# fudan-zvg/S-NeRF

Measured on AMD Instinct MI355X. Metric: rays/sec (train step), higher is better.
Workload: dtype bf16; 1 GPU; S-NeRF path A (MipNerfModel) train step, nuScenes-like 1600x900 rays, 64 proposal + 128 fine evals/ray (192 spp), hidden 1024, rgb_layer 3, cone + contraction + IPE-96

## Files before the change

include/snerf_hip.h:

```cpp
#ifndef SNERF_HIP_H
#define SNERF_HIP_H
#ifdef __cplusplus
extern "C" {
#endif

#define SNERF_DT_F32 0
#define SNERF_DT_BF16 1
#define SNERF_DT_F16 2
#define SNERF_DT_F64 3
#define SNERF_DT_BF16X3 4
#define SNERF_ACT_NONE 0
#define SNERF_ACT_RELU 1
#define SNERF_ACT_MASK 2
#define SNERF_ACT_RELU_BITS 3
#define SNERF_ACT_MASK_BITS 4

int snerf_version(void);
int snerf_last_hip_error(void);
int snerf_debug_lds_scribble(int seed, void* stream);

int snerf_linear_fwd(const void* A, long lda, const void* W, long ldw, const float* bias, void* Y, long ldy,
                     const void* aux, long ldaux, float* colsum, float* colsum_ws, int M, int N, int K, int n_store,
                     int act, int dtype, int out_f32, int variant, void* stream);

// ... 94 lines not shown
                            const float* dirs, long R, int S, int opaque, float bg, float rgb_padding, float density_bias,
                            float* rgb, float* depth, float* acc, float* weights, void* stream);
int snerf_zip_composite_bwd(const float* raw_rgb, long ld_rgb, const float* raw_density, long ld_den, const float* tdist,
                            const float* dirs, long R, int S, int opaque, float bg, float rgb_padding, float density_bias,
                            const float* weights, const float* acc, const float* depth, const float* g_rgb, const float* g_depth,
                            const float* g_acc, const float* g_w, float* d_raw_rgb, long ld_drgb, float* d_raw_density,
                            long ld_dden, float* g_dirs, void* stream);

int snerf_adam_step(float* p, float* g, float* m, float* v, long n, float lr, float b1, float b2, float eps, int step,
                    float grad_scale, int zero_grad, void* stream);
int snerf_app_embed(const float* emb, const float* app, int n_vocab, long n_rays, int S, int dim, void* dst, long ld, int dtype,
                    const int* sample_id, long rows, void* stream);
int snerf_app_embed_bwd(const float* dV, long ld, const float* app, int n_vocab, long n_rays, int S, int dim, float* g_emb, void* stream);
int snerf_app_embed_bwd_det(const float* dV, long ld, const float* app, int n_vocab, long n_rays, int S, int dim, float* g_emb, void* stream);
int snerf_index_check(const float* idx, long n, int n_rows, int* bad, void* stream);

int snerf_split_cast(const float* src, long ld_src, long M, int C, int Cpad, void* dst, long ld_dst, void* stream);

#define SNERF_DT_F16F8 5
int snerf_split8_cast(const float* src, long ld_src, long M, int C, int Cpad, void* dst, long ld_dst, int weight, void* stream);

int snerf_colsum_f32(const float* x, long ld, long M, int C, float* out, void* stream);
int snerf_cast_pad(const float* src, long ld_src, long M, int C, int Cpad, void* dst, long ld_dst, int dtype, void* stream);
int snerf_classic_x_grad(const float* g0, long ld0, const float* g5, long ld5, const float* gv, long ldv, long M, int ic, int icv,
                         float* dx, long ld_dx, void* stream);
int snerf_gather_pack(const float* flat, const int* idx, long n, void* dst, int dtype, void* stream);
int snerf_gather_pack_tiles(const float* flat, const int* idx, long n, void* dst, int dtype, const int* tiles, int n_tiles, void* stream);
int snerf_gather_pack_pair(const float* flat, const int* idx, long n, void* dst, int dtype, const int* tiles, int n_tiles, const int* idx32,
                           long n32, float* dst32, void* stream);

int snerf_semantic_composite_fwd(const float* weights, const void* logits, long ld, int dtype, long R, int S, int C, int softmax,
                                 const int* row_index, float* sem, void* stream);
int snerf_semantic_composite_bwd(const float* weights, const void* logits, long ld, int dtype, const float* g_sem, long R, int S, int C,
                                 int softmax, float* d_logits, long ld_d, float* g_w_out, void* stream);

int snerf_ert_compact(const float* s0, const float* w0, const float* s1, long N, int S0, int S1, float eps_t, float eps_w,
                      void* masks, int* counts, int* row_index, int* sample_id, long* total, void* stream);
int snerf_ert_f2b_step(const float* prev_raw_d, long ld_den, long prev_base, const float* s1, const float* dirs, const float* near,
                       const float* far, long N, int S1, int g0, int G, int next_g0, int next_G, int transform_idx, float density_bias,
                       float eps_t, float* tau, int* flags, int* counts, int* row_index, int* sample_id, long row_base, long* total,
                       void* stream);
int snerf_classic_ert_step(const float* raw_g, int C, const int* alive, long n, const float* z_all, int S, const float* rays, long ld_rays,
                           int g0, int G, float eps_t, float* T, float* raw_full, int* keep, int* offs, int* alive_next, long* total,
                           void* stream);
int snerf_classic_ert_points(const float* rays, long ld_rays, const float* z_all, int S, const int* alive, long n, int g0, int G,
                             float* pts, float* viewdirs, int viewdir_col, void* stream);
// ... 243 lines not shown
```

snerf_amd/_lib.py:

```python
import ctypes
import os
import re

_HERE = os.path.dirname(os.path.abspath(__file__))
_REPO = os.path.dirname(_HERE)
LIB_PATH = os.environ.get("SNERF_HIP_LIB") or os.path.join(_HERE, "lib", "libsnerf_hip.so")
HEADER_PATH = os.path.join(_REPO, "include", "snerf_hip.h")
IO_LIB_PATH = os.path.join(_HERE, "lib", "libsnerf_io.so")
IO_HEADER_PATH = os.path.join(_REPO, "include", "snerf_io.h")

_CTYPE = {"int": ctypes.c_int, "long": ctypes.c_long, "float": ctypes.c_float, "double": ctypes.c_double}
RESTYPE = {}
_lib = None
_iolib = None


def parse_header(path: str = HEADER_PATH):
    src = open(path).read()
    src = re.sub(r"/\*.*?\*/", " ", src, flags=re.S)
    protos = {}
    for m in re.finditer(r"\b(int|long)\s+(snerf_\w+)\s*\(([^)]*)\)\s*;", src):
        name, args = m.group(2), m.group(3).strip()
        RESTYPE[name] = _CTYPE[m.group(1)]
        sig = []
        if args and args != "void":
            for a in args.split(","):
                a = " ".join(a.split())
                if "*" in a:
                    sig.append((ctypes.c_void_p, a.split("*")[-1].strip()))
                else:
                    ty, an = a.rsplit(" ", 1)
                    sig.append((_CTYPE[ty.replace("const ", "").strip()], an))
        protos[name] = sig
    return protos


def load():
    global _lib
    if _lib is not None:
        return _lib
    import torch
    if not os.path.exists(LIB_PATH):
        raise RuntimeError(
            f"libsnerf_hip.so not found at {LIB_PATH}: build it with `python -c 'import __graft_entry__ as g; g.build()'` "
            "(or `make -C snerf_amd/csrc`).  snerf_amd has no CPU/PyTorch fallback for its kernels.")
    lib = ctypes.CDLL(LIB_PATH)
    for name, sig in parse_header().items():
        fn = getattr(lib, name)
        fn.argtypes = [t for t, _ in sig]
        fn.restype = RESTYPE[name]
    _lib = lib
    return lib


def load_io():
    global _iolib
    if _iolib is not None:
        return _iolib
    if not os.path.exists(IO_LIB_PATH):
        raise RuntimeError(f"libsnerf_io.so not found at {IO_LIB_PATH}: build it with `make -C snerf_amd/csrc`")
    lib = ctypes.CDLL(IO_LIB_PATH)
    for name, sig in parse_header(IO_HEADER_PATH).items():
        fn = getattr(lib, name)
        fn.argtypes = [t for t, _ in sig]
        fn.restype = ctypes.c_long if name == "snerf_png_encode" else ctypes.c_int
    _iolib = lib
    return lib


class SnerfHipError(RuntimeError):
    pass


_STATUS = {1: "bad argument", 2: "kernel launch failure"}


def query(name: str, *args):
    return getattr(load(), name)(*args)


def call(name: str, *args):
    rc = getattr(load(), name)(*args)
    if rc != 0:
        extra = f", hipError_t {load().snerf_last_hip_error()}" if rc == 2 else ""
        raise SnerfHipError(f"{name} failed: status {rc} ({_STATUS.get(rc, 'unknown')}{extra})")
```

snerf_amd/csrc/common.h:

```cpp
#pragma once
#include <hip/hip_runtime.h>
#include <stdint.h>

#define SNERF_OK 0
#define SNERF_ERR_ARG 1
#define SNERF_ERR_LAUNCH 2

typedef __attribute__((ext_vector_type(8))) __bf16 bf16x8;
typedef __attribute__((ext_vector_type(4))) __bf16 bf16x4;
typedef __attribute__((ext_vector_type(8))) _Float16 h16x8;
typedef __attribute__((ext_vector_type(16))) float f32x16;
typedef __attribute__((ext_vector_type(4))) float f32x4;

#define SNERF_DT_F32 0
#define SNERF_DT_BF16 1
#define SNERF_DT_F16 2
#define SNERF_DT_F64 3
#define SNERF_DT_BF16X3 4
#define SNERF_DT_F16F8 5

extern int g_snerf_last_hip_error;
static inline int snerf_check_launch() {
  hipError_t e = hipGetLastError();
  if (e != hipSuccess) g_snerf_last_hip_error = (int)e;
  return e == hipSuccess ? SNERF_OK : SNERF_ERR_LAUNCH;
}

template <auto Kernel> static inline void snerf_raise_lds_limit(int limit) {
  static const hipError_t raised = hipFuncSetAttribute((const void*)Kernel, hipFuncAttributeMaxDynamicSharedMemorySize, limit);
  (void)raised;
}
template <auto Kernel, typename... Args>
static inline void snerf_launch(dim3 grid, dim3 block, size_t lds, int limit, hipStream_t stream, const Args&... args) {
  snerf_raise_lds_limit<Kernel>(limit);
  hipLaunchKernelGGL(Kernel, grid, block, lds, stream, args...);
}

static inline int snerf_cu_count() {
  static const int n_cu = [] {
    int dev = 0, n = 0;
    hipDeviceProp_t prop;
    if (hipGetDevice(&dev) == hipSuccess && hipGetDeviceProperties(&prop, dev) == hipSuccess) n = prop.multiProcessorCount;
    return n > 0 ? n : 256;
  }();
  return n_cu;
}

__device__ __forceinline__ int xcd_remap(int bid, int nblk) {
  const int q = nblk >> 3, r = nblk & 7;
  const int xcd = bid & 7, idx = bid >> 3;
  const int base = xcd < r ? xcd * (q + 1) : r * (q + 1) + (xcd - r) * q;
  return base + idx;
}

__device__ __forceinline__ float wave_sum(float v) {
#pragma unroll
  for (int o = 32; o > 0; o >>= 1) v += __shfl_xor(v, o, 64);
  return v;
}
// ... 46 lines not shown
```

snerf_amd/csrc/elementwise.hip:

```cpp
#include "common.h"

struct AdamArgs {
  float lr, b1, b2, eps, grad_scale, grad_max_val;
  int zero_grad, nonfinite;
  const int* step_dev;
  const float* lr_dev;
  const float* clip_coef;
  int step;
  unsigned long long* dropped;
};

__device__ __forceinline__ float adam_clean_grad(float g, const AdamArgs& a, float coef) {
  g *= a.grad_scale * coef;
  if (a.grad_max_val > 0.f && g == g) g = fminf(fmaxf(g, -a.grad_max_val), a.grad_max_val);
  if (a.nonfinite == 1) g = (fabsf(g) <= 3.402823466e+38f) ? g : 0.f;
  else if (a.nonfinite == 2) g = (g != g) ? 0.f : fminf(fmaxf(g, -3.402823466e+38f), 3.402823466e+38f);
  return g;
}

__device__ __forceinline__ void adam_update(float& p, float& m, float& v, float gk, float b1, float b2, float step_size, float bc2_sqrt, float eps) {
#pragma clang fp contract(off)
  m = b1 * m + (1.f - b1) * gk;
  v = b2 * v + ((1.f - b2) * gk) * gk;
  p = p - (step_size * m) / (sqrtf(v) / bc2_sqrt + eps);
// ... 509 lines not shown
      (n_tiles > 0 && (tiles == nullptr || (((uintptr_t)tiles) & 15)))) return SNERF_ERR_ARG;
  if (n_b < 0 || (n_b > 0 && (idx_b == nullptr || dst_b == nullptr || (((uintptr_t)idx_b) & 15)))) return SNERF_ERR_ARG;
  const long want = (n + 1023) / 1024, want_b = (n_b + 1023) / 1024;
  const int gblocks = (int)(want < 4096 ? want : 4096), tblocks = (n_tiles + 3) / 4, bblocks = (int)(want_b < 1024 ? want_b : 1024);
  const dim3 g((unsigned)(gblocks + tblocks + bblocks)), b(256);
  const PackTile* tl = (const PackTile*)tiles;
  hipStream_t s = (hipStream_t)stream;
  if (dtype == SNERF_DT_F32) hipLaunchKernelGGL(gather_pack_tiles_kernel<float>, g, b, 0, s, flat, idx, n, (float*)dst, tl, n_tiles, tblocks, gblocks, idx_b, n_b, dst_b);
  else if (dtype == SNERF_DT_BF16) hipLaunchKernelGGL(gather_pack_tiles_kernel<__bf16>, g, b, 0, s, flat, idx, n, (__bf16*)dst, tl, n_tiles, tblocks, gblocks, idx_b, n_b, dst_b);
  else if (dtype == SNERF_DT_F16) hipLaunchKernelGGL(gather_pack_tiles_kernel<_Float16>, g, b, 0, s, flat, idx, n, (_Float16*)dst, tl, n_tiles, tblocks, gblocks, idx_b, n_b, dst_b);
  else return SNERF_ERR_ARG;
  return snerf_check_launch();
}

extern "C" int snerf_gather_pack_tiles(const float* flat, const int* idx, long n, void* dst, int dtype, const int* tiles, int n_tiles, void* stream) {
  return gather_pack_launch(flat, idx, n, dst, dtype, tiles, n_tiles, nullptr, 0, nullptr, stream);
}

extern "C" int snerf_gather_pack_pair(const float* flat, const int* idx, long n, void* dst, int dtype, const int* tiles, int n_tiles, const int* idx32,
                                      long n32, float* dst32, void* stream) {
  return gather_pack_launch(flat, idx, n, dst, dtype, tiles, n_tiles, idx32, n32, dst32, stream);
}

extern "C" int snerf_version() { return 3; }
int g_snerf_last_hip_error = 0;
extern "C" int snerf_last_hip_error() { return g_snerf_last_hip_error; }

__global__ __launch_bounds__(1024) void lds_scribble_kernel(unsigned seed, unsigned* sink) {
  extern __shared__ unsigned scribble[];
  unsigned h = seed * 2654435761u + blockIdx.x * 40503u + 17u;
  for (int i = threadIdx.x; i < 160 * 1024 / 4; i += 1024) {
    h = (h ^ (unsigned)i) * 1664525u + 1013904223u;
    scribble[i] = (h >> 7) ^ (h << 13);
  }
  __syncthreads();
  if (scribble[(seed + threadIdx.x) % (160 * 1024 / 4)] == 0x5eed5eedu && sink != nullptr) sink[0] = seed;
}
extern "C" int snerf_debug_lds_scribble(int seed, void* stream) {
  snerf_launch<lds_scribble_kernel>(dim3(4096), dim3(1024), 160 * 1024, 160 * 1024, (hipStream_t)stream, (unsigned)seed, (unsigned*)nullptr);
  return snerf_check_launch();
}

__global__ __launch_bounds__(256) void split8_cast_kernel(const float* __restrict__ src, long ld_src, long M, int C, int G, _Float16* __restrict__ dst,
                                                          long ld_dst, int weight) {
  typedef _Float16 f16x8 __attribute__((ext_vector_type(8)));
  typedef unsigned u32x2 __attribute__((ext_vector_type(2)));
  const long total = M * G;
// ... 32 lines not shown
```

snerf_amd/csrc/gemm.hip:

```cpp
#include "common.h"
#include <cstdlib>
#include <type_traits>
#include <utility>

#define ACT_NONE 0
#define ACT_RELU 1
#define ACT_MASK 2
typedef unsigned short u16x2 __attribute__((ext_vector_type(2)));
#define ACT_RELU_BITS 3
#define ACT_MASK_BITS 4

typedef unsigned u32x4 __attribute__((ext_vector_type(4)));
typedef unsigned u32x2 __attribute__((ext_vector_type(2)));

struct GemmNT {
  const void* A; long lda;
  const void* W; long ldw;
  const float* bias;
  void* Y; long ldy;
  const void* aux; long ldaux;
  float* colsum;
  int M, N, K, n_store, act, out_f32, vec_store;
  float* colsum_ws; int fast_epi;
  int det;
// ... 1301 lines not shown
  if (act == ACT_MASK) vec = vec && (ldaux % 4 == 0) && (((uintptr_t)aux) % (dtype == SNERF_DT_F32 ? 16 : 8) == 0);
  if (act >= ACT_RELU_BITS && (((uintptr_t)aux) % 4 != 0)) return SNERF_ERR_ARG;
  const int epc = dtype == SNERF_DT_F32 ? 4 : 8;
  int fast = !(out_f32 && dtype == SNERF_DT_BF16) && (ldy % epc == 0) && (((uintptr_t)Y) % 16 == 0) && (n_store % epc == 0);
  if (act == ACT_MASK) fast = fast && (ldaux % epc == 0) && (((uintptr_t)aux) % 16 == 0);
  if (colsum != nullptr && colsum_ws == nullptr) fast = 0;
  if ((variant >> 4) & 8) fast = 0;
  const int det = (variant >> 8) & 1;
  if (det && colsum != nullptr && !fast) return SNERF_ERR_ARG;
  if (split && !fast && !out_f32) return SNERF_ERR_ARG;
  if (split && out_f32 && (act == ACT_MASK || colsum != nullptr)) return SNERF_ERR_ARG;
  const int aux_split = (variant >> 14) & 1;
  if (aux_split && (split || dtype != SNERF_DT_BF16 || act != ACT_MASK)) return SNERF_ERR_ARG;
  GemmNT p{A, lda, W, ldw, bias, Y, ldy, aux, ldaux, colsum, M, N, K, n_store, act, out_f32, vec, colsum_ws, fast, det, ((variant >> 4) & 7) | ((variant >> 10) & 8),
           (variant >> 9) & 15, split, aux_split};
  variant &= 15;
  hipStream_t s = (hipStream_t)stream;
  const bool p8 = dtype == SNERF_DT_BF16 && (variant & 8) && N % 256 == 0 && K >= 128 && fast && !(colsum != nullptr && act == ACT_RELU) &&
                  (lda * 2 * 256 < (1L << 31)) && (ldw * 2 * 256 < (1L << 31)) && !(split && (act == ACT_MASK || (colsum != nullptr && act == ACT_RELU_BITS))) &&
                  !aux_split &&
                  !(split == 2 && K < 256);
  if (act >= ACT_RELU_BITS && !(p8 && (long)((M + 255) / 256) * 8 * (N / 64) * 256 < (1L << 31)))
    return SNERF_ERR_ARG;
  if (f16) {
    if (p8) return launch_nt8p<true>(p, s);
    if (split == 2) return launch_nt<__bf16, 128, 128, 2, 2, true>(p, s);
    if ((variant & 12) && N % 256 == 0) return launch_nt8<true>(p, s);
    if ((variant & 1) && N % 256 == 0) return launch_nt<__bf16, 256, 256, 2, 4, true>(p, s);
    return launch_nt<__bf16, 128, 128, 2, 2, true>(p, s);
  }
  if (p8) return launch_nt8p(p, s);
  if (dtype == SNERF_DT_BF16 && (variant & 12) && N % 256 == 0) return launch_nt8(p, s);
  if (dtype == SNERF_DT_F32) return launch_nt<float, 128, 128, 2, 2>(p, s);
  if ((variant & 1) && N % 256 == 0) return launch_nt<__bf16, 256, 256, 2, 4>(p, s);
  return launch_nt<__bf16, 128, 128, 2, 2>(p, s);
}

struct GemmTN {
  const void* Z; long ldz;
  const void* X; long ldx;
  float* dW; long ldw;
  const void* zeros;
  int M, N, K, n_valid, k_valid, m_chunk;
  int tiles, slices;
  int split;
  float* part;
// ... 655 lines not shown
```

snerf_amd/mlp.py:

```python
import contextlib

import torch

from . import ops
from .ops import ACT_MASK, ACT_NONE, ACT_RELU, gran, roundup


class ParamArena:

    def __init__(self, shapes, device):
        self.names = [n for n, _ in shapes]
        self.shapes = dict(shapes)
        offs, o = {}, 0
        for n, s in shapes:
            numel = 1
            for d in s:
                numel *= d
            offs[n] = (o, numel)
            o += roundup(numel, 4)
        self.numel = roundup(o, 4)
        self._offs = offs
        self.epoch = 0
        self.flat = torch.zeros(self.numel, dtype=torch.float32, device=device)
        self.grad = torch.zeros(self.numel, dtype=torch.float32, device=device)
# ... 389 lines not shown

    def dgrad(self, key, dZ, K, dX, n_store, mask=None, colsum=None):
        W = self.tw[key]
        bits = getattr(self, "_bits", None)
        if mask is not None and bits:
            ent = bits.get((mask.data_ptr(), mask.shape[0]))
            if ent is not None and ent[1] == W.shape[0] and ops.relu_bits_ok(dZ, W, dX, K, n_store, self.dt, self.variant, consumer=True):
                ops.linear_fwd(dZ, W, None, dX, K, n_store, ops.ACT_MASK_BITS, self.dt, aux=ent[0], colsum=colsum, variant=self.variant,
                               deterministic=self.deterministic)
                return
        act = ACT_MASK if mask is not None else ACT_NONE
        if self.deterministic and colsum is not None and not ops.fast_epilogue_ok(dX, n_store, self.dt, aux=mask, act=act):
            ops.linear_fwd(dZ, W, None, dX, K, n_store, act, self.dt, aux=mask, variant=self.variant, aux_split=getattr(self, "_in_plain_bwd", False) and mask is not None)
            ops.colsum_wide_f32(dX[:, :n_store].float(), n_store, colsum, deterministic=True)
            return
        ops.linear_fwd(dZ, W, None, dX, K, n_store, act, self.dt,
                       aux=mask, colsum=colsum, variant=self.variant, deterministic=self.deterministic,
                       aux_split=getattr(self, "_in_plain_bwd", False) and mask is not None)

    def wgrad(self, name, dZ, X, n_valid, k_valid, wcol=0):
        gw = self.gW(name)
        ops.linear_wgrad(dZ, X, gw[:, wcol:], n_valid, k_valid, self.dt, variant=3,
                         deterministic=self.deterministic, x_split_hi=self._in_plain_bwd)

    def head_grad(self, d_raw_f32, C):
        M = d_raw_f32.shape[0]
        out = self.buf(M, roundup(C, self.g))
        ops.cast_pad(d_raw_f32, C, out, roundup(C, self.g), self.dt)
        return out


class ClassicNeRFNet(_Net):

    def __init__(self, arena, prefix, dt, D=8, W=256, input_ch=63, input_ch_views=27, skips=(4,), variant=8, alpha_head=True, output_ch=0, bwd_plain=False):
        super().__init__(arena, prefix, dt, variant, bwd_plain)
        self.output_ch = int(output_ch)
        assert len(skips) == 1 and 0 <= skips[0] < D - 1 and W % self.g == 0 and (W // 2) % self.g == 0
        self.D, self.Wd, self.ic, self.icv, self.skip = D, W, input_ch, input_ch_views, skips[0]
        self.Pw, self.Vw = roundup(input_ch, self.g), roundup(input_ch_views, self.g)
        self.alpha_head = bool(alpha_head)
        self.fused = True
        self.fused_embed = True
        self.fused_x = True

    @staticmethod
    def param_shapes(D=8, W=256, input_ch=63, input_ch_views=27, skips=(4,), alpha_head=True, output_ch=0):
# ... 398 lines not shown
        M, H = E.shape[0], self.H
        acts, x, k = [], E, self.Ew
        pp = [self.buf(M, H), self.buf(M, H)] if not keep else None
        for i in range(self.L):
            y = self.buf(M, H) if keep else pp[i & 1]
            self.fwd(f"layers.{i}.layers.0", x, k, y, H)
            acts.append((x, k, y))
            x, k = y, H
        out = self.buf(M, 1, f32=True)
        self.fwd("density", x, H, out, 1, ACT_NONE, out_f32=True)
        return out, (acts if keep else None)

    def backward(self, d_raw_density, acts, want_input_grad=False, weight_grads=True):
        with self._bwd():
            if self._fp16_backward():
                return self._scaled_backward([d_raw_density], lambda g: self._backward(g[0], acts, want_input_grad, weight_grads),
                                             weight_grads=weight_grads)
            return self._backward(d_raw_density, acts, want_input_grad, weight_grads)

    def _backward(self, d_raw_density, acts, want_input_grad, weight_grads=True):
        H, M = self.H, d_raw_density.shape[0]
        wg = weight_grads
        gB = self.gB if wg else (lambda name: None)
        if wg:
            self.colsum(d_raw_density, 1, self.gB("density_layer"))
        dz = self.head_grad(d_raw_density, 1)
        xl = acts[-1][2]
        if wg:
            self.wgrad("density_layer", dz, xl, 1, H)
        cb = getattr(self, "_chain_bits", None)
        if cb is not None and cb[0] == acts[0][2].data_ptr() and self.chain_ok():
            dZs = [self.buf(M, H) for _ in range(self.L)]
            ops.fchain_bwd(ops.CHAIN_PROPOSAL, d_raw_density, self._chain_stream(), cb[1], dZs,
                           [self.gB(f"layers.{i}.layers.0") for i in range(self.L - 1, -1, -1)] if wg else self._bias_scratch([H] * self.L))
            for i in range(self.L - 1, -1, -1):
                if wg:
                    self.wgrad(f"layers.{i}.layers.0", dZs[self.L - 1 - i], acts[i][0], H, self.fd if i == 0 else H)
            return self.input_grad("enc", dZs[-1], H, self.Ew) if want_input_grad else None
        dZ = self.buf(M, H)
        self.dgrad("density", dz, self.g, dZ, H, mask=xl, colsum=gB(f"layers.{self.L - 1}.layers.0"))
        for i in range(self.L - 1, -1, -1):
            x, k, y = acts[i]
            n = f"layers.{i}.layers.0"
            if wg:
                self.wgrad(n, dZ, x, H, self.fd if i == 0 else H)
            if i > 0:
                dX = self.buf(M, H)
                self.dgrad(n, dZ, H, dX, H, mask=x, colsum=gB(f"layers.{i - 1}.layers.0"))
                dZ = dX
        return self.input_grad("enc", dZ, H, self.Ew) if want_input_grad else None


class MipNerfNet(_Net):

# ... 140 lines not shown
            self.raw_sem = self.buf(M, self.sc, f32=True)
            self.fwd("sem1", S0, self.Hs, self.raw_sem, self.sc, ACT_NONE, out_f32=True)
        return raw_rgb, raw_d, ((acts, cacts, SKIP, CB, S0) if keep else None)

    def backward(self, d_raw_rgb, d_raw_density, saved, d_raw_sem=None, want_input_grad=False, want_cond_grad=False, on_done=None,
                 weight_grads=True):
        with self._bwd():
            if self._fp16_backward():
                return self._scaled_backward([d_raw_rgb, d_raw_density, d_raw_sem],
                                             lambda g: self._backward(g[0], g[1], saved, g[2], want_input_grad, want_cond_grad, None, weight_grads),
                                             on_done if weight_grads else None, weight_grads=weight_grads)
            return self._backward(d_raw_rgb, d_raw_density, saved, d_raw_sem, want_input_grad, want_cond_grad, on_done, weight_grads)

    def _backward(self, d_raw_rgb, d_raw_density, saved, d_raw_sem=None, want_input_grad=False, want_cond_grad=False, on_done=None,
                  weight_grads=True):
        wg = weight_grads
        gB = self.gB if wg else (lambda name: None)
        if not wg:
            on_done = None
        acts, cacts, SKIP, CB, S0 = saved
        H, g, cu, M = self.H, self.g, self.cu, d_raw_rgb.shape[0]
        dV = None
        DZE = self.buf(M, H * len(self.enc_layers)) if want_input_grad else None
        if wg:
            self.colsum(d_raw_rgb, 3, self.gB("rgb_layer"))
            self.colsum(d_raw_density, 1, self.gB("density_layer"))
        fused = cacts[-1] if (len(cacts) == self.nc + 1 and cacts[-1][0] == "fused") else None
        if fused is not None:
            cacts = cacts[:-1]
        clast = cacts[-1][2]
        if wg or fused is None:
            dz = self.head_grad(d_raw_rgb, 3)
        if wg:
            self.wgrad("rgb_layer", dz, clast, 3, cu)
        DB = self.buf(M, H + g + (self.Hs if self.sc else 0))
        if fused is not None:
            _, cbits, bbits = fused
            dCs = [self.buf(M, cu) for _ in range(self.nc)]
            ops.fcolour_bwd(d_raw_rgb, self._cbwd[0], [cbits[2], cbits[1], cbits[0], bbits], dCs, self.cs(DB, 0, H),
                            [self.gB("cond_layers.2.layers.0"), self.gB("cond_layers.1.layers.0"), self.gB("cond_layers.0.layers.0"),
                             self.gB("bottleneck_layer.layers.0")] if wg else self._bias_scratch([cu] * self.nc + [H]))
            for j in range(self.nc - 1, -1, -1):
                cx, ck, cy = cacts[j]
                if wg:
                    self.wgrad(f"cond_layers.{j}.layers.0", dCs[self.nc - 1 - j], cx, cu, H + self.cd if j == 0 else cu)
            if want_input_grad or want_cond_grad:
                dV = self.input_grad("cenc", dCs[-1], cu, self.Cw)
        else:
            dC = self.buf(M, cu)
            self.dgrad("rgb", dz, g, dC, cu, mask=clast, colsum=gB(f"cond_layers.{self.nc - 1}.layers.0"))
            for j in range(self.nc - 1, -1, -1):
                cx, ck, cy = cacts[j]
                n = f"cond_layers.{j}.layers.0"
                if wg:
                    self.wgrad(n, dC, cx, cu, H + self.cd if j == 0 else cu)
                if j > 0:
                    dX = self.buf(M, cu)
                    self.dgrad(n, dC, cu, dX, cu, mask=cx, colsum=gB(f"cond_layers.{j - 1}.layers.0"))
                    dC = dX
                else:
                    self.dgrad(n, dC, cu, DB, H, mask=CB, colsum=gB("bottleneck_layer.layers.0"))
                    if want_input_grad or want_cond_grad:
                        dV = self.input_grad("cenc", dC, cu, self.Cw)
        ops.cast_pad(d_raw_density, 1, self.cs(DB, H, H + g), g, self.dt)
        xl = acts[-1][2]
        kb = H + g
        if self.sc:
            dS0 = self.cs(DB, H + g)
            if d_raw_sem is None:
                dS0.zero_()
            else:
                if wg:
                    self.colsum(d_raw_sem, self.sc, self.gB("semantic_layer.1"))
                dzs = self.head_grad(d_raw_sem, self.sc)
                if wg:
                    self.wgrad("semantic_layer.1", dzs, S0, self.sc, self.Hs)
                self.dgrad("sem1", dzs, roundup(self.sc, g), dS0, self.Hs, mask=S0, colsum=gB("semantic_layer.0.layers.0"))
                if wg:
                    self.wgrad("semantic_layer.0.layers.0", dS0, xl, self.Hs, H)
            kb += self.Hs
        if wg:
            self.wgrad("bottleneck_layer.layers.0", self.cs(DB, 0, H), xl, H, H)
            self.wgrad("density_layer", self.cs(DB, H, H + g), xl, 1, H)
        dZ = self.buf(M, H)
        self.dgrad("bd", DB, kb, dZ, H, mask=xl, colsum=gB(f"layers.{self.L - 1}.layers.0"))
        if on_done is not None:
            on_done(["density_layer", "bottleneck_layer", "cond_layers", "rgb_layer"] + (["semantic_layer"] if self.sc else []))
        for i in range(self.L - 1, -1, -1):
            x, k, y = acts[i]
            n = f"layers.{i}.layers.0"
            if wg:
                self.wgrad(n, dZ, x, H, self.fd if i == 0 else (H + self.fd if self._is_skip_in(i) else H))
            if on_done is not None:
                on_done([f"layers.{i}."])
            if i > 0:
                xin = acts[i - 1][2]
                if want_input_grad and (i - 1) in self.enc_layers:
                    k = self.enc_layers.index(i - 1)
                    dX = self.cs(DZE, k * H, (k + 1) * H)
                else:
                    dX = self.buf(M, H)
                self.dgrad(n, dZ, H, dX, H, mask=xin, colsum=gB(f"layers.{i - 1}.layers.0"))
                dZ = dX
        if want_input_grad:
            return self.input_grad("enc", DZE, H * len(self.enc_layers), self.Ew), dV
        return dV if want_cond_grad else None
# ... 285 lines not shown
```

snerf_amd/ops.py:

```python
import ctypes
import os as _os

import torch

from . import _lib

F32, BF16, F16, F64 = 0, 1, 2, 3
BF16X3 = 4
F16F8 = 5
SPLIT_DTS = (BF16X3, F16F8)
ACT_NONE, ACT_RELU, ACT_MASK = 0, 1, 2
ACT_RELU_BITS, ACT_MASK_BITS = 3, 4
_TORCH_DT = {F32: torch.float32, BF16: torch.bfloat16, F16: torch.float16, BF16X3: torch.bfloat16, F16F8: torch.float16}


def torch_dtype(dt: int):
    return _TORCH_DT[dt]


def gran(dt: int) -> int:
    return 32 if dt == F32 else 64


def roundup(x: int, m: int) -> int:
    return (x + m - 1) // m * m


def _stream():
    return torch.cuda.current_stream().cuda_stream


def _p(t):
    return None if t is None else t.data_ptr()


def _chk2d(t, dt=None):
    assert t.is_cuda and t.dim() == 2 and t.stride(1) == 1, "expected a row-major 2-D CUDA view"
    if dt is not None:
        assert t.dtype == dt, f"dtype {t.dtype} != {dt}"
    return t


def _f32c(t):
    assert t is None or (t.is_cuda and t.dtype == torch.float32 and t.is_contiguous()), "expected contiguous fp32 CUDA tensor"
    return t


_zeros_cache = {}


def lds_scribble(seed):
    _lib.call("snerf_debug_lds_scribble", int(seed), _stream())


def zero_page(device):
    z = _zeros_cache.get(device)
    if z is None:
        z = torch.zeros(64, dtype=torch.float32, device=device)
        _zeros_cache[device] = z
    return z


# ... 60 lines not shown


def linear_wgrad(dZ, X, dW, n_valid, k_valid, dt, variant=0, deterministic=False, x_split_hi=False):
    _chk2d(dZ, _TORCH_DT[dt]); _chk2d(X, _TORCH_DT[dt]); _chk2d(dW, torch.float32)
    assert dZ.shape[0] == X.shape[0] and dW.shape[0] >= n_valid and dW.shape[1] >= k_valid
    Kx = X.shape[1]
    if x_split_hi:
        assert dt in (BF16, F16) and Kx % 128 == 0
        Kx //= 2
        variant |= 1 << 14
    if dt == BF16X3:
        assert not deterministic, "the split-bf16 weight gradient has no deterministic fold"
        assert dZ.shape[1] % 128 == 0 and X.shape[1] % 128 == 0
    if not deterministic and wgrad_uses_fold(dZ.shape[0], dZ.shape[1], Kx, dt, variant, n_valid, k_valid):
        deterministic = True
    if deterministic:
        nws = _lib.query("snerf_linear_wgrad_ws_floats", dZ.shape[0], dZ.shape[1], Kx, dZ.stride(0), X.stride(0), dt, variant)
        ws = torch.empty(max(int(nws), 1), dtype=torch.float32, device=dZ.device)
        _lib.call("snerf_linear_wgrad_det", _p(dZ), dZ.stride(0), _p(X), X.stride(0), _p(dW), dW.stride(0), _p(zero_page(dZ.device)),
                  dZ.shape[0], dZ.shape[1], Kx, n_valid, k_valid, dt, variant, _p(ws), ws.numel(), _stream())
        return
    _lib.call("snerf_linear_wgrad", _p(dZ), dZ.stride(0), _p(X), X.stride(0), _p(dW), dW.stride(0),
              _p(zero_page(dZ.device)), dZ.shape[0], dZ.shape[1], Kx, n_valid, k_valid, dt, variant, _stream())


def _fmlp_dt(stream):
    assert stream.dtype in (torch.bfloat16, torch.float16) and stream.is_contiguous(), "the fused 256-wide networks run in bf16 or fp16"
    return stream.dtype, _zip_dt(stream)


def fmlp_classic_fwd(E, VE, stream, bias, raw):
    tdt, dt = _fmlp_dt(stream)
    _chk2d(E, tdt); _chk2d(VE, tdt); _chk2d(raw, torch.float32)
    assert bias.dtype == torch.float32 and raw.is_contiguous() and raw.shape[1] == 4
    assert E.shape[1] >= 64 and VE.shape[1] >= 32 and VE.shape[0] == E.shape[0] == raw.shape[0]
    _lib.call("snerf_fmlp_classic_fwd_dt", _p(E), E.stride(0), _p(VE), VE.stride(0), _p(stream), stream.shape[0], _p(bias), bias.numel() // 32,
              _p(raw), E.shape[0], dt, _stream())


def fmlp_classic_pts_fwd(pts, viewdirs, S, stream, bias, raw):
    _f32c(pts); _chk2d(raw, torch.float32)
    _, dt = _fmlp_dt(stream)
    assert viewdirs.dtype == torch.float32 and viewdirs.stride(1) == 1 and viewdirs.shape[1] == 3 and pts.shape[0] == viewdirs.shape[0] * S
    assert bias.dtype == torch.float32 and raw.is_contiguous() and raw.shape == (pts.shape[0], 4)
    _lib.call("snerf_fmlp_classic_pts_fwd_dt", _p(pts), _p(viewdirs), viewdirs.stride(0), int(S), _p(stream), stream.shape[0], _p(bias),
              bias.numel() // 32, _p(raw), pts.shape[0], dt, _stream())
# ... 1574 lines not shown
```

Before: 167,000 rays/s.

## Add GEMV head forward and fused head weight-gradient kernels for narrow output layers

Adds a dedicated GEMV kernel for narrow-output bf16/f16 head layers (n_store<=8) that the generic linear forward dispatches to, instead of a tiled MFMA GEMM padded to 64 columns. Adds a fused head weight-gradient kernel that reads fp32 output grads directly, computes dW and the bias colsum in one pass over slabs, then folds the partials deterministically. This replaces the cast/pad, colsum and padded wgrad launches for the density, rgb and semantic heads, and can skip the head_grad cast when the chain backward is used. The cost is extra workspace and a second reduction launch, and the head math moves to scalar FMA instead of matrix cores.

```diff
diff --git a/include/snerf_hip.h b/include/snerf_hip.h
--- a/include/snerf_hip.h
+++ b/include/snerf_hip.h
@@ -140,6 +140,9 @@
 
 int snerf_colsum_f32(const float* x, long ld, long M, int C, float* out, void* stream);
 int snerf_cast_pad(const float* src, long ld_src, long M, int C, int Cpad, void* dst, long ld_dst, int dtype, void* stream);
+long snerf_head_wgrad_ws_floats(long M, int C, int K);
+int snerf_head_wgrad(const float* d, long ldd, const void* X, long ldx, float* dW, long ldw, float* dB, long M, int C, int K, int k_valid,
+                     int dtype, float* ws, long ws_floats, void* stream);
 int snerf_classic_x_grad(const float* g0, long ld0, const float* g5, long ld5, const float* gv, long ldv, long M, int ic, int icv,
                          float* dx, long ld_dx, void* stream);
 int snerf_gather_pack(const float* flat, const int* idx, long n, void* dst, int dtype, void* stream);
diff --git a/snerf_amd/_lib.py b/snerf_amd/_lib.py
--- a/snerf_amd/_lib.py
+++ b/snerf_amd/_lib.py
@@ -10,6 +10,7 @@
 IO_HEADER_PATH = os.path.join(_REPO, "include", "snerf_io.h")
 
 _CTYPE = {"int": ctypes.c_int, "long": ctypes.c_long, "float": ctypes.c_float, "double": ctypes.c_double}
+OPTIONAL = {"snerf_head_wgrad", "snerf_head_wgrad_ws_floats"}
 RESTYPE = {}
 _lib = None
 _iolib = None
@@ -46,6 +47,8 @@
             "(or `make -C snerf_amd/csrc`).  snerf_amd has no CPU/PyTorch fallback for its kernels.")
     lib = ctypes.CDLL(LIB_PATH)
     for name, sig in parse_header().items():
+        if name in OPTIONAL and not hasattr(lib, name):
+            continue
         fn = getattr(lib, name)
         fn.argtypes = [t for t, _ in sig]
         fn.restype = RESTYPE[name]
@@ -75,6 +78,10 @@
 _STATUS = {1: "bad argument", 2: "kernel launch failure"}
 
 
+def has(name: str) -> bool:
+    return hasattr(load(), name)
+
+
 def query(name: str, *args):
     return getattr(load(), name)(*args)
 
diff --git a/snerf_amd/csrc/common.h b/snerf_amd/csrc/common.h
--- a/snerf_amd/csrc/common.h
+++ b/snerf_amd/csrc/common.h
@@ -35,6 +35,10 @@
   snerf_raise_lds_limit<Kernel>(limit);
   hipLaunchKernelGGL(Kernel, grid, block, lds, stream, args...);
 }
+
+bool snerf_head_fwd_takes(const void* A, long lda, const void* W, long ldw, int N, int K, int n_store);
+int snerf_head_fwd_launch(const void* A, long lda, const void* W, long ldw, const float* bias, float* Y, long ldy, long M, int K, int n_store,
+                          bool f16, hipStream_t stream);
 
 static inline int snerf_cu_count() {
   static const int n_cu = [] {
diff --git a/snerf_amd/csrc/elementwise.hip b/snerf_amd/csrc/elementwise.hip
--- a/snerf_amd/csrc/elementwise.hip
+++ b/snerf_amd/csrc/elementwise.hip
@@ -555,7 +555,7 @@
   return gather_pack_launch(flat, idx, n, dst, dtype, tiles, n_tiles, idx32, n32, dst32, stream);
 }
 
-extern "C" int snerf_version() { return 3; }
+extern "C" int snerf_version() { return 4; }
 int g_snerf_last_hip_error = 0;
 extern "C" int snerf_last_hip_error() { return g_snerf_last_hip_error; }
 
diff --git a/snerf_amd/csrc/gemm.hip b/snerf_amd/csrc/gemm.hip
--- a/snerf_amd/csrc/gemm.hip
+++ b/snerf_amd/csrc/gemm.hip
@@ -1347,6 +1347,9 @@
                   !(split == 2 && K < 256);
   if (act >= ACT_RELU_BITS && !(p8 && (long)((M + 255) / 256) * 8 * (N / 64) * 256 < (1L << 31)))
     return SNERF_ERR_ARG;
+  if (!split && dtype == SNERF_DT_BF16 && act == ACT_NONE && out_f32 && n_store <= 8 && colsum == nullptr && aux == nullptr &&
+      snerf_head_fwd_takes(A, lda, W, ldw, N, K, n_store))
+    return snerf_head_fwd_launch(A, lda, W, ldw, bias, (float*)Y, ldy, M, K, n_store, f16, s);
   if (f16) {
     if (p8) return launch_nt8p<true>(p, s);
     if (split == 2) return launch_nt<__bf16, 128, 128, 2, 2, true>(p, s);
diff --git a/snerf_amd/csrc/head.hip b/snerf_amd/csrc/head.hip
--- /dev/null
+++ b/snerf_amd/csrc/head.hip
@@ -0,0 +1,253 @@
+#include "common.h"
+#include <stdlib.h>
+
+template <typename T> struct Vec8;
+template <> struct Vec8<__bf16> { typedef bf16x8 type; };
+template <> struct Vec8<_Float16> { typedef h16x8 type; };
+
+template <typename T, int NS>
+__global__ __launch_bounds__(256) void head_gemv_fwd_kernel(const T* __restrict__ A, long lda, const T* __restrict__ W, long ldw,
+                                                             const float* __restrict__ bias, float* __restrict__ Y, long ldy, long M, int K,
+                                                             int n_store) {
+  typedef typename Vec8<T>::type vec8;
+  extern __shared__ __attribute__((aligned(16))) char smem[];
+  T* sW = (T*)smem;
+  const int kc = K >> 3;
+  for (int c = threadIdx.x; c < NS * kc; c += 256) {
+    const int j = c / kc, q = c - j * kc;
+    *(vec8*)(sW + (long)j * K + q * 8) = *(const vec8*)(W + (long)j * ldw + q * 8);
+  }
+  __syncthreads();
+  const int l8 = threadIdx.x & 7, rsub = threadIdx.x >> 3;
+  const int steps = K >> 6;
+  const long groups = (M + 31) >> 5;
+  for (long g = blockIdx.x; g < groups; g += gridDim.x) {
+    const long row = g * 32 + rsub;
+    const T* a = A + (row < M ? row : M - 1) * lda + l8 * 8;
+    const T* w = sW + l8 * 8;
+    float acc[NS];
+#pragma unroll
+    for (int j = 0; j < NS; ++j) acc[j] = 0.f;
+    int s = 0;
+    for (; s + 4 <= steps; s += 4) {
+      vec8 x[4];
+#pragma unroll
+      for (int u = 0; u < 4; ++u) x[u] = *(const vec8*)(a + (s + u) * 64);
+#pragma unroll
+      for (int u = 0; u < 4; ++u)
+#pragma unroll
+        for (int j = 0; j < NS; ++j) {
+          const vec8 wv = *(const vec8*)(w + (long)j * K + (s + u) * 64);
+#pragma unroll
+          for (int e = 0; e < 8; ++e) acc[j] = fmaf((float)x[u][e], (float)wv[e], acc[j]);
+        }
+    }
+    for (; s < steps; ++s) {
+      const vec8 x = *(const vec8*)(a + s * 64);
+#pragma unroll
+      for (int j = 0; j < NS; ++j) {
+        const vec8 wv = *(const vec8*)(w + (long)j * K + s * 64);
+#pragma unroll
+        for (int e = 0; e < 8; ++e) acc[j] = fmaf((float)x[e], (float)wv[e], acc[j]);
+      }
+    }
+#pragma unroll
+    for (int j = 0; j < NS; ++j) {
+      acc[j] += __shfl_xor(acc[j], 1, 64);
+      acc[j] += __shfl_xor(acc[j], 2, 64);
+      acc[j] += __shfl_xor(acc[j], 4, 64);
+    }
+    if (l8 == 0 && row < M) {
+#pragma unroll
+      for (int j = 0; j < NS; ++j)
+        if (j < n_store) Y[row * ldy + j] = acc[j] + (bias != nullptr ? bias[j] : 0.f);
+    }
+  }
+}
+
+static bool head_gemv_enabled() {
+  const char* e = getenv("SNERF_HEAD_GEMV");
+  return e == nullptr || atoi(e) != 0;
+}
+
+template <typename T, int NS>
+static int head_fwd_go(const void* A, long lda, const void* W, long ldw, const float* bias, float* Y, long ldy, long M, int K, int n_store,
+                       hipStream_t stream) {
+  const long groups = (M + 31) / 32;
+  const long cap = (long)snerf_cu_count() * 8;
+  const int grid = (int)(groups < cap ? groups : cap);
+  const int lds = NS * K * 2;
+  hipLaunchKernelGGL((head_gemv_fwd_kernel<T, NS>), dim3(grid), dim3(256), lds, stream, (const T*)A, lda, (const T*)W, ldw, bias, Y, ldy, M, K,
+                     n_store);
+  return snerf_check_launch();
+}
+
+bool snerf_head_fwd_takes(const void* A, long lda, const void* W, long ldw, int N, int K, int n_store) {
+  if (!head_gemv_enabled() || n_store < 1 || n_store > 8) return false;
+  const int ns = n_store <= 1 ? 1 : (n_store <= 2 ? 2 : (n_store <= 4 ? 4 : 8));
+  return N >= ns && K % 64 == 0 && (long)ns * K * 2 <= 65536 && lda % 8 == 0 && ldw % 8 == 0 && (((uintptr_t)A) & 15) == 0 && (((uintptr_t)W) & 15) == 0;
+}
+
+int snerf_head_fwd_launch(const void* A, long lda, const void* W, long ldw, const float* bias, float* Y, long ldy, long M, int K, int n_store,
+                          bool f16, hipStream_t stream) {
+#define HEAD_FWD(NS) (f16 ? head_fwd_go<_Float16, NS>(A, lda, W, ldw, bias, Y, ldy, M, K, n_store, stream) \
+                          : head_fwd_go<__bf16, NS>(A, lda, W, ldw, bias, Y, ldy, M, K, n_store, stream))
+  if (n_store <= 1) return HEAD_FWD(1);
+  if (n_store <= 2) return HEAD_FWD(2);
+  if (n_store <= 4) return HEAD_FWD(4);
+  return HEAD_FWD(8);
+#undef HEAD_FWD
+}
+
+template <typename T, int NC>
+__global__ __launch_bounds__(256) void head_wgrad_kernel(const float* __restrict__ d, long ldd, const T* __restrict__ X, long ldx, long M, int C,
+                                                          int K, long slab_rows, float* __restrict__ ws, long ws_stride) {
+  typedef typename Vec8<T>::type vec8;
+  extern __shared__ __attribute__((aligned(16))) float red[];
+  const int g8 = K >> 3;
+  const int gw = g8 < 256 ? g8 : 256;
+  const int per = 256 / gw;
+  const int cl = threadIdx.x % gw, rsub = threadIdx.x / gw;
+  const int cg = cl + blockIdx.y * 256;
+  const bool live = cg < g8 && rsub < per;
+  const bool bias_thread = cl == 0 && blockIdx.y == 0;
+  const long r0 = (long)blockIdx.x * slab_rows, r1 = r0 + slab_rows < M ? r0 + slab_rows : M;
+  float acc[NC][8], bacc[NC];
+#pragma unroll
+  for (int j = 0; j < NC; ++j) {
+    bacc[j] = 0.f;
+#pragma unroll
+    for (int e = 0; e < 8; ++e) acc[j][e] = 0.f;
+  }
+  if (live) {
+    const T* x = X + (long)cg * 8;
+    long r = r0 + rsub;
+    for (; r + 3L * per < r1; r += 4L * per) {
+      vec8 xv[4];
+      float dv[4][NC];
+#pragma unroll
+      for (int u = 0; u < 4; ++u) {
+        xv[u] = *(const vec8*)(x + (r + (long)u * per) * ldx);
+#pragma unroll
+        for (int j = 0; j < NC; ++j) dv[u][j] = j < C ? d[(r + (long)u * per) * ldd + j] : 0.f;
+      }
+#pragma unroll
+      for (int u = 0; u < 4; ++u)
+#pragma unroll
+        for (int j = 0; j < NC; ++j) {
+          const float dr = (float)(T)dv[u][j];
+          bacc[j] += dv[u][j];
+#pragma unroll
+          for (int e = 0; e < 8; ++e) acc[j][e] = fmaf(dr, (float)xv[u][e], acc[j][e]);
+        }
+    }
+    for (; r < r1; r += per) {
+      const vec8 xv = *(const vec8*)(x + r * ldx);
+#pragma unroll
+      for (int j = 0; j < NC; ++j) {
+        const float dj = j < C ? d[r * ldd + j] : 0.f;
+        const float dr = (float)(T)dj;
+        bacc[j] += dj;
+#pragma unroll
+        for (int e = 0; e < 8; ++e) acc[j][e] = fmaf(dr, (float)xv[e], acc[j][e]);
+      }
+    }
+  }
+  const int w8 = gw * 8;
+  float* bred = red + per * NC * w8;
+  if (rsub < per) {
+#pragma unroll
+    for (int j = 0; j < NC; ++j) {
+      *(f32x4*)(red + ((long)rsub * NC + j) * w8 + cl * 8) = f32x4{acc[j][0], acc[j][1], acc[j][2], acc[j][3]};
+      *(f32x4*)(red + ((long)rsub * NC + j) * w8 + cl * 8 + 4) = f32x4{acc[j][4], acc[j][5], acc[j][6], acc[j][7]};
+      if (bias_thread) bred[rsub * 8 + j] = bacc[j];
+    }
+  }
+  __syncthreads();
+  float* out = ws + (long)blockIdx.x * ws_stride;
+  for (int i = threadIdx.x; i < NC * w8; i += 256) {
+    const int j = i / w8, c = i - j * w8;
+    const int k = blockIdx.y * 2048 + c;
+    if (k >= K) continue;
+    float s = 0.f;
+    for (int q = 0; q < per; ++q) s += red[((long)q * NC + j) * w8 + c];
+    out[(long)j * K + k] = s;
+  }
+  if (blockIdx.y == 0 && threadIdx.x < 8) {
+    float s = 0.f;
+    if (threadIdx.x < NC)
+      for (int q = 0; q < per; ++q) s += bred[q * 8 + threadIdx.x];
+    out[(long)NC * K + threadIdx.x] = s;
+  }
+}
+
+__global__ __launch_bounds__(1024) void head_wgrad_fold_kernel(const float* __restrict__ ws, long ws_stride, int slabs, int NC, int C, int K,
+                                                                int k_valid, float* __restrict__ dW, long ldw, float* __restrict__ dB) {
+  __shared__ float red[64][16];
+  const int o = threadIdx.x & 15, grp = threadIdx.x >> 4;
+  const int total = NC * K + 8;
+  const int i = blockIdx.x * 16 + o;
+  const int share = (slabs + 63) / 64;
+  float s = 0.f;
+  if (i < total) {
+    const int s0 = grp * share, s1 = s0 + share < slabs ? s0 + share : slabs;
+    for (int q = s0; q < s1; ++q) s += ws[(long)q * ws_stride + i];
+  }
+  red[grp][o] = s;
+  __syncthreads();
+  if (threadIdx.x < 16 && i < total) {
+    float t = 0.f;
+    for (int q = 0; q < 64; ++q) t += red[q][o];
+    if (i < NC * K) {
+      const int j = i / K, k = i - j * K;
+      if (j < C && k < k_valid) dW[(long)j * ldw + k] += t;
+    } else if (i - NC * K < C && dB != nullptr) dB[i - NC * K] += t;
+  }
+}
+
+static int head_wgrad_nc(int C) { return C <= 1 ? 1 : (C <= 2 ? 2 : (C <= 4 ? 4 : 8)); }
+static int head_wgrad_per(int K) { const int g8 = K / 8; return 256 / (g8 < 256 ? g8 : 256); }
+static long head_wgrad_slabs(long M, int K) {
+  const long rows_min = 4L * head_wgrad_per(K);
+  long slabs = (M + rows_min - 1) / rows_min;
+  return slabs > 1024 ? 1024 : (slabs < 1 ? 1 : slabs);
+}
+
+extern "C" long snerf_head_wgrad_ws_floats(long M, int C, int K) {
+  if (M <= 0 || C < 1 || C > 8 || K < 64 || K % 8 != 0) return 0;
+  return head_wgrad_slabs(M, K) * ((long)head_wgrad_nc(C) * K + 8);
+}
+
+template <typename T, int NC>
+static void head_wgrad_go(const float* d, long ldd, const void* X, long ldx, long M, int C, int K, long slabs, long slab_rows, float* ws,
+                          long ws_stride, hipStream_t stream) {
+  const int g8 = K / 8, gw = g8 < 256 ? g8 : 256, per = 256 / gw;
+  const int lds = (per * NC * gw * 8 + per * 8) * 4;
+  snerf_launch<head_wgrad_kernel<T, NC>>(dim3((unsigned)slabs, (g8 + 255) / 256), dim3(256), lds, 8 * 256 * 8 * 4 + 32 * 8 * 4, stream, d, ldd,
+                                         (const T*)X, ldx, M, C, K, slab_rows, ws, ws_stride);
+}
+
+extern "C" int snerf_head_wgrad(const float* d, long ldd, const void* X, long ldx, float* dW, long ldw, float* dB, long M, int C, int K,
+                                int k_valid, int dtype, float* ws, long ws_floats, void* stream) {
+  if (M <= 0) return SNERF_OK;
+  if (d == nullptr || X == nullptr || dW == nullptr || ws == nullptr) return SNERF_ERR_ARG;
+  if (C < 1 || C > 8 || K < 64 || K % 8 != 0 || k_valid < 0 || k_valid > K || ldd < C || ldx < K || ldx % 8 != 0 || ldw < k_valid) return SNERF_ERR_ARG;
+  if (dtype != SNERF_DT_BF16 && dtype != SNERF_DT_F16) return SNERF_ERR_ARG;
+  if ((((uintptr_t)X) & 15) != 0 || (((uintptr_t)d) & 3) != 0 || (((uintptr_t)ws) & 15) != 0) return SNERF_ERR_ARG;
+  if (ws_floats < snerf_head_wgrad_ws_floats(M, C, K)) return SNERF_ERR_ARG;
+  const int NC = head_wgrad_nc(C), per = head_wgrad_per(K);
+  const long slabs = head_wgrad_slabs(M, K);
+  long slab_rows = (M + slabs - 1) / slabs;
+  slab_rows = (slab_rows + per - 1) / per * per;
+  const long ws_stride = (long)NC * K + 8;
+  hipStream_t s = (hipStream_t)stream;
+  const bool f16 = dtype == SNERF_DT_F16;
+#define HEAD_WG(N_) (f16 ? head_wgrad_go<_Float16, N_>(d, ldd, X, ldx, M, C, K, slabs, slab_rows, ws, ws_stride, s) \
+                         : head_wgrad_go<__bf16, N_>(d, ldd, X, ldx, M, C, K, slabs, slab_rows, ws, ws_stride, s))
+  if (NC == 1) HEAD_WG(1); else if (NC == 2) HEAD_WG(2); else if (NC == 4) HEAD_WG(4); else HEAD_WG(8);
+#undef HEAD_WG
+  const int total = NC * K + 8;
+  hipLaunchKernelGGL(head_wgrad_fold_kernel, dim3((total + 15) / 16), dim3(1024), 0, s, (const float*)ws, ws_stride, (int)slabs, NC, C, K, k_valid, dW,
+                     ldw, dB);
+  return snerf_check_launch();
+}
diff --git a/snerf_amd/mlp.py b/snerf_amd/mlp.py
--- a/snerf_amd/mlp.py
+++ b/snerf_amd/mlp.py
@@ -435,6 +435,12 @@
         gw = self.gW(name)
         ops.linear_wgrad(dZ, X, gw[:, wcol:], n_valid, k_valid, self.dt, variant=3,
                          deterministic=self.deterministic, x_split_hi=self._in_plain_bwd)
+
+    def head_stream_ok(self):
+        return ops.HEAD_GEMV and self.dt in (ops.BF16, ops.F16) and not self._in_plain_bwd
+
+    def head_wgrad(self, name, d_raw_f32, X, C, k_valid):
+        ops.head_wgrad(d_raw_f32, X, self.gW(name), self.gB(name), C, k_valid, self.dt, deterministic=self.deterministic)
 
     def head_grad(self, d_raw_f32, C):
         M = d_raw_f32.shape[0]
@@ -879,14 +885,19 @@
         H, M = self.H, d_raw_density.shape[0]
         wg = weight_grads
         gB = self.gB if wg else (lambda name: None)
-        if wg:
+        xl = acts[-1][2]
+        cb = getattr(self, "_chain_bits", None)
+        chain = cb is not None and cb[0] == acts[0][2].data_ptr() and self.chain_ok()
+        hs = self.head_stream_ok()
+        if wg and hs:
+            self.head_wgrad("density_layer", d_raw_density, xl, 1, H)
+        elif wg:
             self.colsum(d_raw_density, 1, self.gB("density_layer"))
-        dz = self.head_grad(d_raw_density, 1)
-        xl = acts[-1][2]
-        if wg:
+        if not (hs and chain):
+            dz = self.head_grad(d_raw_density, 1)
+        if wg and not hs:
             self.wgrad("density_layer", dz, xl, 1, H)
-        cb = getattr(self, "_chain_bits", None)
-        if cb is not None and cb[0] == acts[0][2].data_ptr() and self.chain_ok():
+        if chain:
             dZs = [self.buf(M, H) for _ in range(self.L)]
             ops.fchain_bwd(ops.CHAIN_PROPOSAL, d_raw_density, self._chain_stream(), cb[1], dZs,
                            [self.gB(f"layers.{i}.layers.0") for i in range(self.L - 1, -1, -1)] if wg else self._bias_scratch([H] * self.L))
@@ -1073,16 +1084,19 @@
         H, g, cu, M = self.H, self.g, self.cu, d_raw_rgb.shape[0]
         dV = None
         DZE = self.buf(M, H * len(self.enc_layers)) if want_input_grad else None
-        if wg:
+        hs = self.head_stream_ok()
+        if wg and not hs:
             self.colsum(d_raw_rgb, 3, self.gB("rgb_layer"))
             self.colsum(d_raw_density, 1, self.gB("density_layer"))
         fused = cacts[-1] if (len(cacts) == self.nc + 1 and cacts[-1][0] == "fused") else None
         if fused is not None:
             cacts = cacts[:-1]
         clast = cacts[-1][2]
-        if wg or fused is None:
+        if (wg and not hs) or fused is None:
             dz = self.head_grad(d_raw_rgb, 3)
-        if wg:
+        if wg and hs:
+            self.head_wgrad("rgb_layer", d_raw_rgb, clast, 3, cu)
+        elif wg:
             self.wgrad("rgb_layer", dz, clast, 3, cu)
         DB = self.buf(M, H + g + (self.Hs if self.sc else 0))
         if fused is not None:
@@ -1121,10 +1135,13 @@
             if d_raw_sem is None:
                 dS0.zero_()
             else:
-                if wg:
+                hss = hs and self.sc <= 8
+                if wg and not hss:
                     self.colsum(d_raw_sem, self.sc, self.gB("semantic_layer.1"))
                 dzs = self.head_grad(d_raw_sem, self.sc)
-                if wg:
+                if wg and hss:
+                    self.head_wgrad("semantic_layer.1", d_raw_sem, S0, self.sc, self.Hs)
+                elif wg:
                     self.wgrad("semantic_layer.1", dzs, S0, self.sc, self.Hs)
                 self.dgrad("sem1", dzs, roundup(self.sc, g), dS0, self.Hs, mask=S0, colsum=gB("semantic_layer.0.layers.0"))
                 if wg:
@@ -1132,7 +1149,10 @@
             kb += self.Hs
         if wg:
             self.wgrad("bottleneck_layer.layers.0", self.cs(DB, 0, H), xl, H, H)
-            self.wgrad("density_layer", self.cs(DB, H, H + g), xl, 1, H)
+            if hs:
+                self.head_wgrad("density_layer", d_raw_density, xl, 1, H)
+            else:
+                self.wgrad("density_layer", self.cs(DB, H, H + g), xl, 1, H)
         dZ = self.buf(M, H)
         self.dgrad("bd", DB, kb, dZ, H, mask=xl, colsum=gB(f"layers.{self.L - 1}.layers.0"))
         if on_done is not None:
diff --git a/snerf_amd/ops.py b/snerf_amd/ops.py
--- a/snerf_amd/ops.py
+++ b/snerf_amd/ops.py
@@ -38,6 +38,11 @@
     assert t.is_cuda and t.dim() == 2 and t.stride(1) == 1, "expected a row-major 2-D CUDA view"
     if dt is not None:
         assert t.dtype == dt, f"dtype {t.dtype} != {dt}"
+    return t
+
+
+def _chk2d_any(t, dt):
+    assert t.dim() == 2 and t.stride(1) == 1 and t.dtype == dt, "expected a row-major 2-D view"
     return t
 
 
@@ -144,6 +149,29 @@
         return
     _lib.call("snerf_linear_wgrad", _p(dZ), dZ.stride(0), _p(X), X.stride(0), _p(dW), dW.stride(0),
               _p(zero_page(dZ.device)), dZ.shape[0], dZ.shape[1], Kx, n_valid, k_valid, dt, variant, _stream())
+
+
+HEAD_GEMV = _os.environ.get("SNERF_HEAD_GEMV", "1") != "0"
+
+
+def head_wgrad(d, X, dW, dB, C, k_valid, dt, deterministic=False):
+    assert dt in (BF16, F16) and 1 <= C <= 8
+    _chk2d_any(d, torch.float32); _chk2d_any(X, _TORCH_DT[dt]); _chk2d_any(dW, torch.float32)
+    M, K = X.shape
+    assert d.shape[0] == M and d.shape[1] >= C and dW.shape[0] >= C and dW.shape[1] >= k_valid and k_valid <= K
+    if not d.is_cuda or not _lib.has("snerf_head_wgrad"):
+        if dB is not None:
+            colsum_f32(d, C, dB, deterministic=deterministic)
+        g = gran(dt)
+        dz = torch.empty(M, roundup(C, g), dtype=_TORCH_DT[dt], device=d.device)
+        cast_pad(d, C, dz, roundup(C, g), dt)
+        linear_wgrad(dz, X, dW, C, k_valid, dt, variant=3, deterministic=deterministic)
+        return
+    assert dB is None or (dB.is_cuda and dB.dtype == torch.float32 and dB.is_contiguous() and dB.numel() >= C)
+    nws = _lib.query("snerf_head_wgrad_ws_floats", M, C, K)
+    ws = torch.empty(max(int(nws), 1), dtype=torch.float32, device=d.device)
+    _lib.call("snerf_head_wgrad", _p(d), d.stride(0), _p(X), X.stride(0), _p(dW), dW.stride(0), _p(dB), M, C, K, k_valid, dt, _p(ws), ws.numel(),
+              _stream())
 
 
 def _fmlp_dt(stream):
```

After: 168,300 rays/s, median of 6. No clear change (+0.8%).
